# graehl/carmel

Hardware: AMD Instinct MI355X
Metric: arc-updates/sec (EM iterations/sec x derivation-lattice arcs swept per iteration) (higher is better)
Workload: dtype f64; 1 GPU; c4: synthetic 1000000-state / 9999990-arc WFST, 1000000 training pairs per GPU (random walks of 5-40 arcs), conditional normalisation, cached lattices; parallelism=corpus-sharded x1, none

## Files before the change

### carmel_amd/csrc/engine.cpp

```cpp
#include <hip/hip_runtime.h>
#include <chrono>
#include <cmath>
#include <cstdio>
#include <cstring>
#include <cstdlib>
#include <limits>
#include <string>
#include <thread>
#include <unordered_map>
#include <vector>
#include "engine.hpp"
#include "options.hpp"
#include "host/refhash.hpp"
#include "rng.hpp"
#include "unrolled_args.hpp"

int unrolled_try_build(carmel_hip_trainer* t, int host_threads, uint8_t* has_derivation, carmel_hip_lattice_stats* stats);
int gpu_build_lattices(carmel_hip_trainer* t, const BuildOptions& opt, uint8_t* has_derivation, carmel_hip_lattice_stats* stats,
                       bool& done);
int gpu_tables_for_host_layout(carmel_hip_trainer* t, const std::vector<uint32_t>& lane_arc, const std::vector<uint32_t>& wave_arc);
int carmel_hip_debug_lattice_fingerprint_impl(carmel_hip_trainer* t, uint64_t* out);
int build_run_tables(carmel_hip_trainer* t);
int exchange_weights_in(carmel_hip_trainer* t, ExchangePlan* xp, const TransArgs& T, bool need_x);
int exchange_counts_out(carmel_hip_trainer* t, ExchangePlan* xp, const TransArgs& T);
// ... 828 lines not shown
  T.b_src = t->t_b_src.p;
  T.t_pos = t->t_t_pos.p;
  T.t_src = t->t_t_src.p;
  T.a_off = t->t_a_off.p;
  T.tr_off = t->tr_off.p;
  T.tr_rel = t->tr_rel.p;
  T.tr_src = t->tr_src.p;
  T.br_off = t->br_off.p;
  T.br_rel = t->br_rel.p;
  T.br_src = t->br_src.p;
  T.use_runs = t->use_runs ? 1u : 0u;
  {
    const char* e = lib_opt("trans_scatter");
    T.scatter = e ? (uint32_t)atoi(e) : (t->use_runs ? 3u : 0u);
    if (t->lat.lane_fused) T.scatter &= ~2u;
  }
  T.x = t->t_x.p;
  T.xc = t->t_xc.p;
  T.logw = t->arc_logw.p;
  T.wcache = t->wcache.p;
  T.post = t->post.p;
  T.counts = t->counts_ptr();
  T.n_wcache = t->wcache.n;
  T.n_post = t->post.n;
  T.n_buckets = (uint32_t)t->t_buckets.n;
  T.n_tiles = t->t_tile_base.n ? (uint32_t)(t->t_tile_base.n - 1) : 0u;
  T.tile = t->lat.tile;
  T.bucket = t->lat.bucket;
  T.tile_first = T.tile_count = 0;
  T.bucket_first = 0;
  T.bucket_count = T.n_buckets;
  T.n_wtiles = 0;
  T.slack_bytes = (uint32_t)DEVBUF_SLACK;
}

__global__ __launch_bounds__(256) void lds_poison_kernel(unsigned* sink) {
  extern __shared__ unsigned lds_words[];
  const unsigned n = 160 * 1024 / 4 - 64;
  for (unsigned i = threadIdx.x; i < n; i += 256) lds_words[i] = 0xffffffffu;
  __syncthreads();
  if (lds_words[(threadIdx.x * 977u) % n] != 0xffffffffu) *sink = 1;
}
static int lds_poison(carmel_hip_trainer* t) {
  const int mode = lib_opt("poison") ? atoi(lib_opt("poison")) : 0;
  if (mode < 2) return CARMEL_HIP_OK;
  static bool attr = false;
  const int bytes = 160 * 1024 - 256;
  if (!attr) {
    HIPCHK(hipFuncSetAttribute((const void*)lds_poison_kernel, hipFuncAttributeMaxDynamicSharedMemorySize, bytes));
    attr = true;
  }
  hipLaunchKernelGGL(lds_poison_kernel, dim3(2048), dim3(256), bytes, t->stream, (unsigned*)t->maxchg.p);
  HIPCHK(hipGetLastError());
  HIPCHK(hipStreamSynchronize(t->stream));
  return CARMEL_HIP_OK;
}

int scalars_join(carmel_hip_trainer* t) {
  if (!t->scalars_pending) return CARMEL_HIP_OK;
  if (hipEventQuery(t->ev_join) != hipSuccess) HIPCHK(hipStreamWaitEvent(t->stream, t->ev_join, 0));
  t->scalars_pending = false;
  return CARMEL_HIP_OK;
}

__global__ void publish_kernel(const unsigned long long* src, unsigned long long* box, unsigned long long seq) {
  __hip_atomic_store(box, *src, __ATOMIC_RELAXED, __HIP_MEMORY_SCOPE_SYSTEM);
// ... 742 lines not shown
```

### carmel_amd/csrc/kernels.hip

```cpp
#include "kernels.hpp"
#include "sweep_math.hpp"
#include <algorithm>
#include <cstdio>
#include <cstdlib>

namespace carmel_hip {


__device__ __forceinline__ double lw_add(double a, double b) {
  if (a == NEG_INF) return b;
  if (b == NEG_INF) return a;
  double d = a - b;
  if (d > 36.0) return a;
  if (d < -36.0) return b;
  if (d < 0) return b + log1p(exp(d));
  return a + log1p(exp(-d));
}

__device__ __forceinline__ void atomic_add_f64(double* p, double v) {
  unsafeAtomicAdd(p, v);
}


#define LANE_W(r) (PRE ? wcache[(size_t)(((r).x >> LANE_POS_SHIFT) & LANE_POS_MAX) * 64] : logw[(r).y])
// ... 521 lines not shown
    f[s] = NEG_INF;
    bb[s] = NEG_INF;
  }
  f[st] = 0.0;
  for (uint32_t s = 0; s < ns; ++s) {
    for (uint32_t a = ooff[s]; a < ooff[s + 1]; ++a) {
      const uint2 r = oa[a];
      f[r.x] = lw_add(f[r.x], f[s] + A.logw[r.y]);
    }
  }
  const double prob = f[fin];
  A.pair_logprob[A.pair_id[d.pair_base]] = prob;
  const double lwt = A.pair_logw[d.pair_base];
  bb[fin] = 0.0;
  for (uint32_t s = ns; s-- > 0;) {
    for (uint32_t a = ioff[s]; a < ioff[s + 1]; ++a) {
      const uint2 r = ia[a];
      bb[r.x] = lw_add(bb[r.x], bb[s] + A.logw[r.y]);
    }
  }
  for (uint32_t s = 0; s < ns; ++s)
    for (uint32_t a = ooff[s]; a < ooff[s + 1]; ++a) {
      const uint2 r = oa[a];
      post[a] = (prob != NEG_INF) ? exp(A.logw[r.y] + f[s] + bb[r.x] + lwt - prob) : 0.0;
    }
}

#define SCALAR_BLOCKS 256
__global__ __launch_bounds__(256) void scalars_partial_kernel(const double* __restrict__ pair_logprob,
                                                              const double* __restrict__ pair_w, uint64_t n_pairs,
                                                              double* __restrict__ partial) {
  __shared__ double sh[3][4];
  double a = 0.0, b = 0.0, c = 0.0;
  for (uint64_t p = (uint64_t)blockIdx.x * 256 + threadIdx.x; p < n_pairs; p += (uint64_t)SCALAR_BLOCKS * 256) {
    const double w = pair_w[p];
    if (w < 0.0) continue;
    const double lp = pair_logprob[p];
    a += lp;
    b += lp * w;
    c += 1.0;
  }
  for (int o = 32; o > 0; o >>= 1) {
    a += __shfl_down(a, o, 64);
    b += __shfl_down(b, o, 64);
    c += __shfl_down(c, o, 64);
  }
  if ((threadIdx.x & 63) == 0) {
    sh[0][threadIdx.x >> 6] = a;
    sh[1][threadIdx.x >> 6] = b;
    sh[2][threadIdx.x >> 6] = c;
  }
  __syncthreads();
  if (threadIdx.x < 3) partial[blockIdx.x * 3 + threadIdx.x] = sh[threadIdx.x][0] + sh[threadIdx.x][1] + sh[threadIdx.x][2] + sh[threadIdx.x][3];
}
__global__ void scalars_final_kernel(const double* __restrict__ partial, double* __restrict__ scalars) {
  if (threadIdx.x < 3) {
    double v[4] = {0.0, 0.0, 0.0, 0.0};
    for (int k = 0; k < SCALAR_BLOCKS; k += 4)
      for (int j = 0; j < 4; ++j) v[j] += partial[(k + j) * 3 + threadIdx.x];
    scalars[threadIdx.x] = (v[0] + v[1]) + (v[2] + v[3]);
  } else if (threadIdx.x == 3)
    scalars[3] = 0.0;
}

#define COUNT_HOT 64
__global__ __launch_bounds__(256) void count_reduce_kernel(ReduceArgs R) {
  for (uint64_t a = (uint64_t)blockIdx.x * blockDim.x + threadIdx.x; a < R.n_arcs;
       a += (uint64_t)gridDim.x * blockDim.x) {
    const uint64_t j0 = R.arc_off[a], j1 = R.arc_off[a + 1];
    double c = 0.0;
    if (j1 - j0 <= COUNT_HOT)
      for (uint64_t j = j0; j < j1; ++j) c += R.post[R.slot_pos[j]];
    R.counts[a] = c;
// ... 330 lines not shown
                                     const double* arc_prior_w, const uint32_t* arc_chain, const uint64_t* chain_off,
                                     const uint64_t* chain_param, const uint32_t* param_group, uint64_t n_arcs) {
  for (uint64_t k = (uint64_t)blockIdx.x * blockDim.x + threadIdx.x; k < n_arcs; k += (uint64_t)gridDim.x * blockDim.x) {
    const double c = arc_counts[k] + (arc_prior_w ? arc_prior + arc_prior_w[k] : arc_prior);
    if (!(c > 0.0)) continue;
    const uint32_t ch = arc_chain[k];
    for (uint64_t j = chain_off[ch]; j < chain_off[ch + 1]; ++j) {
      const uint64_t p = chain_param[j];
      if (param_group[p] != 0u) atomic_add_f64(param_counts + p, c);
    }
  }
}

__global__ void add_f64_kernel(double* dst, const double* src, uint64_t n) {
  for (uint64_t k = (uint64_t)blockIdx.x * blockDim.x + threadIdx.x; k < n; k += (uint64_t)gridDim.x * blockDim.x) dst[k] += src[k];
}
__global__ void fill_f64_kernel(double* p, double v, uint64_t n) {
  for (uint64_t k = (uint64_t)blockIdx.x * blockDim.x + threadIdx.x; k < n; k += (uint64_t)gridDim.x * blockDim.x) p[k] = v;
}

#define TRANS_RUN_WORDS ((TRANS_TILE > TRANS_BUCKET ? TRANS_TILE : TRANS_BUCKET) / 32)
struct RunLds {
  uint32_t* r_src;
  uint32_t* mask;
  uint32_t* pref;
};
__device__ __forceinline__ RunLds run_lds(double* after_tile) {
  RunLds R;
  R.r_src = (uint32_t*)after_tile;
  R.mask = R.r_src + TRANS_RUN_CAP;
  R.pref = R.mask + TRANS_RUN_WORDS;
  return R;
}
__device__ __forceinline__ void run_stage(const RunLds& R, const uint16_t* __restrict__ rel, const uint32_t* __restrict__ src,
                                          uint32_t nr) {
  constexpr uint32_t WORDS = TRANS_RUN_WORDS, PER = WORDS / 64;
  for (uint32_t w = threadIdx.x; w < WORDS; w += 1024) R.mask[w] = 0u;
  __syncthreads();
  for (uint32_t r = threadIdx.x; r < nr; r += 1024) {
    const uint32_t first = rel[r];
    R.r_src[r] = src[r] - first;
    atomicOr(&R.mask[first >> 5], 1u << (first & 31u));
  }
  __syncthreads();
  if (threadIdx.x < 64) {
    uint32_t c[PER], tot = 0;
#pragma unroll
    for (uint32_t k = 0; k < PER; ++k) {
      c[k] = tot;
      tot += __popc(R.mask[threadIdx.x * PER + k]);
    }
    uint32_t inc = tot;
#pragma unroll
    for (int o = 1; o < 64; o <<= 1) {
      const uint32_t v = __shfl_up(inc, o, 64);
      if ((int)threadIdx.x >= o) inc += v;
    }
    const uint32_t before = inc - tot;
#pragma unroll
    for (uint32_t k = 0; k < PER; ++k) R.pref[threadIdx.x * PER + k] = before + c[k];
  }
  __syncthreads();
}
__device__ __forceinline__ uint32_t run_source(const RunLds& R, uint32_t i) {
  const uint32_t w = i >> 5;
  const uint32_t run = R.pref[w] + __popc(R.mask[w] & (0xffffffffu >> (31u - (i & 31u)))) - 1u;
  return R.r_src[run] + i;
}
template <bool SC, bool RL, int KB = TRANS_KB>
__global__ __launch_bounds__(1024) void trans_w_bucket_kernel(TransArgs T) {
  extern __shared__ __attribute__((aligned(16))) double lds[];
  const RunLds R = run_lds(lds + KB * 1024);
  uint32_t bloc = blockIdx.x;
  if (SC) {
    bloc = xcd_chunked(blockIdx.x, T.bucket_count);
    if (bloc >= T.bucket_count) return;
  }
  const uint32_t bucket = T.bucket_first + bloc;
  const TransBucket B = T.buckets[bucket];
  double w[KB];
#pragma unroll
  for (int k = 0; k < KB; ++k) {
    const uint32_t a = threadIdx.x + k * 1024;
    w[k] = a < B.n_arcs ? T.logw[B.arc_lo + a] : 0.0;
  }
  uint16_t ia[KB];
  uint32_t dst[KB];
#pragma unroll
  for (int k = 0; k < KB; ++k) {
    const uint32_t j = threadIdx.x + k * 1024;
    ia[k] = j < B.n_items ? T.b_arc[B.item_base + j] : (uint16_t)0;
    if (SC && !RL) dst[k] = j < B.n_items ? T.b_src[B.item_base + j] : 0u;
  }
#pragma unroll
  for (int k = 0; k < KB; ++k) lds[threadIdx.x + k * 1024] = w[k];
  if (SC && RL) {
    const uint32_t r0 = T.br_off[bucket];
    run_stage(R, T.br_rel + r0, T.br_src + r0, T.br_off[bucket + 1] - r0);
  } else
    __syncthreads();
#pragma unroll
  for (int k = 0; k < KB; ++k) {
    const uint32_t j = threadIdx.x + k * 1024;
    if (j < B.n_items) {
      if (SC)
        T.x[RL ? run_source(R, j) : dst[k]] = lds[ia[k]];
      else
        T.x[B.item_base + j] = lds[ia[k]];
    }
  }
}
#ifndef TRANS_TILE_WAVES
#define TRANS_TILE_WAVES 4
#endif
#ifndef TRANS_WB_WAVES
#define TRANS_WB_WAVES 4
#endif
template <bool RL, bool SQ>
__global__ __launch_bounds__(1024) __attribute__((amdgpu_waves_per_eu(TRANS_TILE_WAVES, TRANS_TILE_WAVES))) void trans_w_tile_kernel(TransArgs T) {
  extern __shared__ __attribute__((aligned(16))) double lds[];
  const RunLds R = run_lds(lds + TRANS_TILE);
  const uint32_t tloc = xcd_chunked(blockIdx.x, T.tile_count);
  if (tloc >= T.tile_count) return;
  const uint32_t tile = T.tile_first + tloc;
  const uint64_t p0 = (uint64_t)tile * T.tile;
  if (p0 >= T.n_wcache) return;
  const uint32_t np = (uint32_t)min((uint64_t)T.tile, T.n_wcache - p0);
#pragma unroll
  for (int k = 0; k < TRANS_KT; ++k) lds[threadIdx.x + k * 1024] = 0.0;
  if (RL && !SQ) {
    const uint32_t r0 = T.tr_off[tile];
    run_stage(R, T.tr_rel + r0, T.tr_src + r0, T.tr_off[tile + 1] - r0);
// ... 114 lines not shown
    if (threadIdx.x + k * NT < ni) lds[pos[k]] = v[k];
  __syncthreads();
#pragma unroll
  for (int k = 0; k < K; ++k) {
    const uint32_t q = threadIdx.x + k * NT;
    if (q < np) T.wcache[p0 + q] = lds[q];
  }
}
__global__ __launch_bounds__(TRANS_SMALL_THREADS) void trans_c_tile_small_kernel(TransArgs T) {
  __shared__ double lds[LANE_FUSED_TILE];
  constexpr int NT = TRANS_SMALL_THREADS, K = TRANS_SMALL_K;
  const uint32_t tile = T.tile_first + blockIdx.x;
  const uint64_t p0 = (uint64_t)tile * LANE_FUSED_TILE;
  const uint32_t np = p0 < T.n_post ? (uint32_t)min((uint64_t)LANE_FUSED_TILE, T.n_post - p0) : 0u;
  const uint64_t i0 = T.tile_base[tile];
  const uint32_t ni = (uint32_t)(T.tile_base[tile + 1] - i0);
  double v[K];
  uint16_t pos[K];
#pragma unroll
  for (int k = 0; k < K; ++k) {
    const uint32_t q = threadIdx.x + k * NT;
    v[k] = q < np ? T.post[p0 + q] : 0.0;
    pos[k] = q < ni ? T.t_pos[i0 + q] : (uint16_t)0;
  }
#pragma unroll
  for (int k = 0; k < K; ++k) lds[threadIdx.x + k * NT] = v[k];
  __syncthreads();
#pragma unroll
  for (int k = 0; k < K; ++k) {
    const uint32_t i = threadIdx.x + k * NT;
    if (i < ni) T.xc[i0 + i] = lds[pos[k]];
  }
}
template <bool RL, bool SQ, int KB = TRANS_KB>
__global__ __launch_bounds__(1024) void trans_c_bucket_kernel(TransArgs T) {
  extern __shared__ __attribute__((aligned(16))) double lds[];
  const RunLds R = run_lds(lds + KB * 1024);
  __shared__ double part[16];
  __shared__ uint32_t big[512];
  __shared__ uint32_t n_big;
  const uint32_t bloc = xcd_chunked(blockIdx.x, T.bucket_count);
  if (bloc >= T.bucket_count) return;
  const uint32_t bucket = T.bucket_first + bloc;
  const TransBucket B = T.buckets[bucket];
  uint16_t r0[KB], r1[KB];
  const bool single = (B.flags & TRANS_SINGLE) != 0;
#pragma unroll
  for (int k = 0; k < KB; ++k) {
    const uint32_t a = threadIdx.x + k * 1024;
    const bool ok = !single && a < B.n_arcs;
    r0[k] = ok ? T.a_off[B.arc_lo + a] : (uint16_t)0;
    r1[k] = (ok && a + 1 < B.n_arcs) ? T.a_off[B.arc_lo + a + 1] : (uint16_t)0;
  }
  {
    uint32_t src[KB];
    uint16_t rk[KB];
    double v[KB];
    if (RL && !SQ) {
      const uint32_t r0 = T.br_off[bucket];
      run_stage(R, T.br_rel + r0, T.br_src + r0, T.br_off[bucket + 1] - r0);
    }
#pragma unroll
    for (int k = 0; k < KB; ++k) {
      const uint32_t j = threadIdx.x + k * 1024;
      if (SQ)
        src[k] = 0u;
      else if (RL)
        src[k] = j < B.n_items ? run_source(R, j) : 0u;
      else
        src[k] = j < B.n_items ? T.b_src[B.item_base + j] : 0u;
      rk[k] = j < B.n_items ? T.b_rank[B.item_base + j] : (uint16_t)0;
    }
#pragma unroll
    for (int k = 0; k < KB; ++k) {
      if (SQ) {
        const uint32_t j = threadIdx.x + k * 1024;
        v[k] = j < B.n_items ? T.xc[B.item_base + j] : 0.0;
      } else
        v[k] = T.xc[src[k]];
    }
#pragma unroll
    for (int k = 0; k < KB; ++k)
      if (threadIdx.x + k * 1024 < B.n_items) lds[rk[k]] = v[k];
  }
  __syncthreads();
  if (single) {
    double v = 0.0;
    for (uint32_t j = threadIdx.x; j < B.n_items; j += 1024) v += lds[j];
    for (int o = 32; o > 0; o >>= 1) v += __shfl_down(v, o, 64);
    if ((threadIdx.x & 63) == 0) part[threadIdx.x >> 6] = v;
    __syncthreads();
    if (threadIdx.x == 0) {
      double tot = 0.0;
      for (int k = 0; k < 16; ++k) tot += part[k];
      if (B.flags & TRANS_SPLIT)
        atomic_add_f64(T.counts + B.arc_lo, tot);
      else
        T.counts[B.arc_lo] = tot;
    }
    return;
  }
  if (threadIdx.x == 0) n_big = 0;
  __syncthreads();
#pragma unroll
  for (int k = 0; k < KB; ++k) {
    const uint32_t a = threadIdx.x + k * 1024;
    if (a >= B.n_arcs) break;
    const uint32_t q0 = r0[k], q1 = a + 1 < B.n_arcs ? (uint32_t)r1[k] : B.n_items;
    if (q1 - q0 > 32) {
      const uint32_t q = atomicAdd(&n_big, 1u);
      if (q < 512) {
        big[q] = a;
        continue;
      }
    }
    double v = 0.0;
    for (uint32_t r = q0; r < q1; ++r) v += lds[r];
    T.counts[B.arc_lo + a] = v;
  }
  __syncthreads();
  const uint32_t nb = n_big < 512 ? n_big : 512;
  for (uint32_t q = threadIdx.x >> 6; q < nb; q += 16) {
    const uint32_t a = big[q];
    const uint32_t q0 = T.a_off[B.arc_lo + a], q1 = a + 1 < B.n_arcs ? (uint32_t)T.a_off[B.arc_lo + a + 1] : B.n_items;
    double v = 0.0;
    for (uint32_t r = q0 + (threadIdx.x & 63); r < q1; r += 64) v += lds[r];
    for (int o = 32; o > 0; o >>= 1) v += __shfl_down(v, o, 64);
    if ((threadIdx.x & 63) == 0) T.counts[B.arc_lo + a] = v;
  }
}
__global__ void zero_list_kernel(double* p, const uint32_t* idx, uint32_t n) {
  uint32_t k = blockIdx.x * blockDim.x + threadIdx.x;
  if (k < n) p[idx[k]] = 0.0;
}

static inline int grid_for(uint64_t n, int block) {
  uint64_t g = (n + block - 1) / block;
  if (g > 256ull * 16) g = 256ull * 16;
  if (g < 1) g = 1;
  return (int)g;
}

template <int R, int W, bool PRE, bool WIN = false, bool XC = false>
static hipError_t launch_lane_variant(const LaneArgs& A, unsigned grid, size_t lds, hipStream_t stream) {
  if (lds > 64 * 1024)
    (void)hipFuncSetAttribute((const void*)sweep_lane_kernel<R, W, PRE, Lse, WIN, XC>, hipFuncAttributeMaxDynamicSharedMemorySize, (int)lds);
  hipLaunchKernelGGL((sweep_lane_kernel<R, W, PRE, Lse, WIN, XC>), dim3(grid), dim3(64), lds, stream, A);
  return hipGetLastError();
}

hipError_t launch_lane_sweep(const LaneArgs& A0, const LatticeSet::LaneClass& lc, hipStream_t stream, bool fused) {
  LaneArgs A = A0;
  A.first_group = lc.first;
  A.lds_rows = lc.max_states;
  size_t lds = (size_t)lc.max_states * 64 * sizeof(double);
  if (fused) {
    if (!A.pre_weights || !A.xc || !A.xc_tile_base || !A.xc_t_pos) return hipErrorInvalidValue;
    lds += (size_t)LANE_FUSED_TILE * sizeof(double);
    if (lc.windowed) {
      if (!A.spill) return hipErrorInvalidValue;
      return launch_lane_variant<4, 2, true, true, true>(A, lc.count, lds, stream);
// ... 62 lines not shown
  } else if (lc.block == 64) {
    hipLaunchKernelGGL((sweep_bundle_kernel<64, true>), dim3(lc.count), dim3(64), lds, stream, A);
  } else if (lc.block == 256) {
    hipLaunchKernelGGL((sweep_bundle_kernel<256, true>), dim3(lc.count), dim3(256), lds, stream, A);
  } else {
    (void)hipFuncSetAttribute((const void*)sweep_bundle_kernel<1024, true>, hipFuncAttributeMaxDynamicSharedMemorySize,
                              (int)lds);
    hipLaunchKernelGGL((sweep_bundle_kernel<1024, true>), dim3(lc.count), dim3(1024), lds, stream, A);
  }
  return hipGetLastError();
}

#define TRANS_SET_LDS(K, BYTES) (void)hipFuncSetAttribute((const void*)K, hipFuncAttributeMaxDynamicSharedMemorySize, BYTES)
static void trans_lds_attr() {
  static unsigned char done_dev[64] = {0};
  int dev = 0;
  if (hipGetDevice(&dev) != hipSuccess || dev < 0 || dev >= 64) return;
  unsigned char& done = done_dev[dev];
  if (__atomic_load_n(&done, __ATOMIC_ACQUIRE)) return;
  const int lds = (int)(TRANS_TILE > TRANS_BUCKET ? TRANS_TILE : TRANS_BUCKET) * 8;
  const int lds_rl = lds + TRANS_RUN_LDS;
  TRANS_SET_LDS((trans_w_bucket_kernel<false, false>), lds);
  TRANS_SET_LDS((trans_w_bucket_kernel<true, false>), lds);
  TRANS_SET_LDS((trans_w_bucket_kernel<true, true>), lds_rl);
  TRANS_SET_LDS((trans_w_tile_kernel<false, false>), lds);
  TRANS_SET_LDS((trans_w_tile_kernel<true, false>), lds_rl);
  TRANS_SET_LDS((trans_w_tile_kernel<false, true>), lds);
  TRANS_SET_LDS((trans_c_tile_kernel<false, false>), lds);
  TRANS_SET_LDS((trans_c_tile_kernel<true, false>), lds);
  TRANS_SET_LDS((trans_c_tile_kernel<true, true>), lds_rl);
  TRANS_SET_LDS((trans_c_bucket_kernel<false, false>), lds);
  TRANS_SET_LDS((trans_c_bucket_kernel<true, false>), lds_rl);
  TRANS_SET_LDS((trans_c_bucket_kernel<false, true>), lds);
  {
    constexpr int KH = TRANS_KB / 2;
    TRANS_SET_LDS((trans_w_bucket_kernel<false, false, KH>), lds);
    TRANS_SET_LDS((trans_w_bucket_kernel<true, false, KH>), lds);
    TRANS_SET_LDS((trans_w_bucket_kernel<true, true, KH>), lds_rl);
    TRANS_SET_LDS((trans_c_bucket_kernel<false, false, KH>), lds);
    TRANS_SET_LDS((trans_c_bucket_kernel<true, false, KH>), lds_rl);
    TRANS_SET_LDS((trans_c_bucket_kernel<false, true, KH>), lds);
  }
  __atomic_store_n(&done, (unsigned char)1, __ATOMIC_RELEASE);
}
hipError_t launch_trans_w_bucket_range(const TransArgs& T0, uint32_t first, uint32_t count, hipStream_t stream) {
  trans_lds_attr();
  if (!T0.n_buckets || !count) return hipSuccess;
  TransArgs T = T0;
  T.bucket_first = first;
  T.bucket_count = count;
  const dim3 g8((count + 7) / 8 * 8);
  if (T.bucket == TRANS_BUCKET / 2) {
    constexpr int KH = TRANS_KB / 2;
    if (!(T.scatter & 1u))
      hipLaunchKernelGGL((trans_w_bucket_kernel<false, false, KH>), dim3(count), dim3(1024), KH * 1024 * 8, stream, T);
    else if (T.use_runs)
      hipLaunchKernelGGL((trans_w_bucket_kernel<true, true, KH>), g8, dim3(1024), KH * 1024 * 8 + TRANS_RUN_LDS, stream, T);
    else
      hipLaunchKernelGGL((trans_w_bucket_kernel<true, false, KH>), g8, dim3(1024), KH * 1024 * 8, stream, T);
    return hipGetLastError();
  }
  if (T.bucket != TRANS_BUCKET) return hipErrorInvalidValue;
  if (!(T.scatter & 1u))
    hipLaunchKernelGGL((trans_w_bucket_kernel<false, false>), dim3(count), dim3(1024), TRANS_BUCKET * 8, stream, T);
  else if (T.use_runs)
    hipLaunchKernelGGL((trans_w_bucket_kernel<true, true>), g8, dim3(1024), TRANS_BUCKET * 8 + TRANS_RUN_LDS, stream, T);
  else
    hipLaunchKernelGGL((trans_w_bucket_kernel<true, false>), g8, dim3(1024), TRANS_BUCKET * 8, stream, T);
  return hipGetLastError();
}
hipError_t launch_trans_w_bucket(const TransArgs& T, hipStream_t stream) { return launch_trans_w_bucket_range(T, 0, T.n_buckets, stream); }
hipError_t launch_trans_w_tiles(const TransArgs& T0, uint32_t tile_first, uint32_t tile_count, hipStream_t stream) {
  trans_lds_attr();
  if (!T0.n_buckets || !tile_count) return hipSuccess;
  TransArgs T = T0;
  T.tile_first = tile_first;
// ... 28 lines not shown
    return hipGetLastError();
  }
  if (T.tile != TRANS_TILE && T.tile != TILE_SWEEP_TILE) return hipErrorInvalidValue;
  if (!(T.scatter & 2u))
    hipLaunchKernelGGL((trans_c_tile_kernel<false, false>), dim3(tile_count), dim3(1024), TRANS_TILE * 8, stream, T);
  else if (T.use_runs)
    hipLaunchKernelGGL((trans_c_tile_kernel<true, true>), g8, dim3(1024), TRANS_TILE * 8 + TRANS_RUN_LDS, stream, T);
  else
    hipLaunchKernelGGL((trans_c_tile_kernel<true, false>), g8, dim3(1024), TRANS_TILE * 8, stream, T);
  return hipGetLastError();
}
hipError_t launch_zero_list(double* p, const uint32_t* idx, uint32_t n, hipStream_t stream) {
  if (n) hipLaunchKernelGGL(zero_list_kernel, dim3((n + 255) / 256), dim3(256), 0, stream, p, idx, n);
  return hipGetLastError();
}
hipError_t launch_trans_c_bucket_range(const TransArgs& T0, uint32_t first, uint32_t count, hipStream_t stream) {
  trans_lds_attr();
  if (!T0.n_buckets || !count) return hipSuccess;
  TransArgs T = T0;
  T.bucket_first = first;
  T.bucket_count = count;
  const dim3 g8((count + 7) / 8 * 8);
  if (T.bucket == TRANS_BUCKET / 2) {
    constexpr int KH = TRANS_KB / 2;
    if (T.scatter & 2u)
      hipLaunchKernelGGL((trans_c_bucket_kernel<false, true, KH>), g8, dim3(1024), KH * 1024 * 8, stream, T);
    else if (T.use_runs)
      hipLaunchKernelGGL((trans_c_bucket_kernel<true, false, KH>), g8, dim3(1024), KH * 1024 * 8 + TRANS_RUN_LDS, stream, T);
    else
      hipLaunchKernelGGL((trans_c_bucket_kernel<false, false, KH>), g8, dim3(1024), KH * 1024 * 8, stream, T);
    return hipGetLastError();
  }
  if (T.bucket != TRANS_BUCKET) return hipErrorInvalidValue;
  if (T.scatter & 2u)
    hipLaunchKernelGGL((trans_c_bucket_kernel<false, true>), g8, dim3(1024), TRANS_BUCKET * 8, stream, T);
  else if (T.use_runs)
    hipLaunchKernelGGL((trans_c_bucket_kernel<true, false>), g8, dim3(1024), TRANS_BUCKET * 8 + TRANS_RUN_LDS, stream, T);
  else
    hipLaunchKernelGGL((trans_c_bucket_kernel<false, false>), g8, dim3(1024), TRANS_BUCKET * 8, stream, T);
  return hipGetLastError();
}
hipError_t launch_trans_c_bucket(const TransArgs& T, const uint32_t* split_arcs, uint32_t n_split, hipStream_t stream) {
  if (!T.n_buckets) return hipSuccess;
  hipError_t e = launch_zero_list(T.counts, split_arcs, n_split, stream);
  if (e != hipSuccess) return e;
  return launch_trans_c_bucket_range(T, 0, T.n_buckets, stream);
}
__global__ void gather_idx_kernel(double* small, const double* src, const uint32_t* idx, uint32_t n) {
  const uint32_t k = blockIdx.x * blockDim.x + threadIdx.x;
  if (k < n) small[k] = src[idx[k]];
}
__global__ void scatter_idx_kernel(double* dst, const double* small, const uint32_t* idx, uint32_t n) {
  const uint32_t k = blockIdx.x * blockDim.x + threadIdx.x;
  if (k < n) dst[idx[k]] = small[k];
}
hipError_t launch_gather_idx(double* small, const double* src, const uint32_t* idx, uint32_t n, hipStream_t stream) {
  if (n) hipLaunchKernelGGL(gather_idx_kernel, dim3((n + 255) / 256), dim3(256), 0, stream, small, src, idx, n);
  return hipGetLastError();
}
hipError_t launch_scatter_idx(double* dst, const double* small, const uint32_t* idx, uint32_t n, hipStream_t stream) {
  if (n) hipLaunchKernelGGL(scatter_idx_kernel, dim3((n + 255) / 256), dim3(256), 0, stream, dst, small, idx, n);
  return hipGetLastError();
}

hipError_t launch_count_reduce(const ReduceArgs& R, hipStream_t stream) {
  if (!R.n_arcs) return hipSuccess;
// ... 103 lines not shown
```

### carmel_amd/csrc/kernels.hpp

```cpp
#pragma once
#include <hip/hip_runtime.h>
#include <stdint.h>
#include "lattice.hpp"

namespace carmel_hip {

struct LaneArgs {
  const LaneGroup* groups;
  const uint2* fwd;
  const uint32_t* fwdx;
  const uint32_t* bwd;
  const uint32_t* rec2;
  const uint32_t* chain;
  const uint32_t* tile_chain;
  const uint32_t* lane_pair;
  const uint32_t* lane_nstates;
  const double* lane_logw;
  const double* logw;
  double* post;
  double* wcache;
  double* scalars;
  double* pair_logprob;
  double* spill;
  uint32_t first_group;
// ... 57 lines not shown
struct TransArgs {
  const TransBucket* buckets;
  const uint64_t* tile_base;
  const uint16_t* b_arc;
  const uint16_t* b_rank;
  const uint32_t* b_src;
  const uint16_t* t_pos;
  const uint32_t* t_src;
  const uint16_t* a_off;
  double* x;
  double* xc;
  const double* logw;
  double* wcache;
  const double* post;
  double* counts;
  uint64_t n_wcache, n_post;
  uint32_t n_buckets, n_tiles;
  uint32_t n_wtiles;
  const uint32_t* tr_off;
  const uint16_t* tr_rel;
  const uint32_t* tr_src;
  const uint32_t* br_off;
  const uint16_t* br_rel;
  const uint32_t* br_src;
  uint32_t use_runs;
  uint32_t scatter;
  uint32_t tile;
  uint32_t bucket;
  uint32_t tile_first, tile_count;
  uint32_t bucket_first, bucket_count;
  uint32_t slack_bytes;
  const uint32_t* zero_list = nullptr;
  uint32_t n_zero = 0;
};

#define TRANS_RUN_CAP 4096
#define TRANS_RUN_LDS (TRANS_RUN_CAP * 4 + 4096)
#define MSTEP_BIG_GROUP 48
#define MSTEP_PARTIALS 2048
#define MSTEP_MAX_RANGES 17
#define MSTEP_WIDE_SLOTS 512
#define MSTEP_WIDE_SHARDS 32
#define MSTEP_WIDE_TICKETS (16 * (MSTEP_WIDE_SHARDS + 1))
struct MstepArgs {
  double* logw;
  const double* lw_src;
  double* old_logw;
  const double* counts;
  const double* prior;
  const uint32_t* group;
  const uint32_t* norm_of;
  const double* add_count;
  const uint64_t* group_off;
  const uint64_t* norm_perm;
  const uint64_t* big_groups;
  uint64_t n_groups, n_big;
  double* gscale;
  unsigned long long* max_partial;
  unsigned long long* max_change_bits;
  int all_grouped;
  uint32_t window_span;
  double* glocked;
  const uint32_t* tie_of;
  double* tie_tab;
  uint64_t n_ties;
  uint64_t n;
  uint32_t block_first;
// ... 57 lines not shown
```

### carmel_amd/csrc/options.cpp

```cpp
#include "options.hpp"
#include <cstdlib>
#include <cstring>
#include <mutex>
#include <string>
#include "../../include/carmel_hip.h"

namespace carmel_hip {
namespace {
const char* const kKeys[] = {
    "timing",
    "lane_states", "tile_sweep", "lane_fused", "transpose", "lane_chunks", "lane_window", "lane_window_min", "wave_ring", "wave_min_width",
    "gpu_build", "wave_gather", "wave_xc", "tile_gather", "device_tables", "trans_scatter", "trans_runs", "lane_fused_kernel",
    "tile_sweep_kernel", "mailbox", "poison", "lane_trace", "exchange_sparse", "mstep_wide",
    "dense", "unrolled", "unrolled_ragged",
    "gibbs_chains", "gibbs_own_cap", "gibbs_workgroup", "gibbs_clk", "gibbs_reg", "gibbs_lane", "forest_sweep", "forest_ldswalk", "forest_multi",
    "forest_nohash", "forest_trace", "forest_exact_host", "forest_exact_clk", "forest_logdomain", "forest_gcol", "forest_gather",
    "decode_lds", "decode_chunk_bytes"};
constexpr int kN = (int)(sizeof kKeys / sizeof kKeys[0]);
const char* volatile g_val[kN];
std::mutex g_mu;
int find(const char* key) {
  for (int i = 0; i < kN; ++i)
    if (!std::strcmp(kKeys[i], key)) return i;
  return -1;
}
}
const char* lib_opt(const char* key) {
  const int i = find(key);
  return i < 0 ? nullptr : g_val[i];
}
bool lib_opt_off(const char* key) {
  const char* v = lib_opt(key);
  return v && std::atoi(v) == 0;
}
}

extern "C" {
int carmel_hip_set_option(const char* key, const char* value) {
  using namespace carmel_hip;
  if (!key) return CARMEL_HIP_ERR_ARG;
  const int i = find(key);
  if (i < 0) return CARMEL_HIP_ERR_ARG;
  std::lock_guard<std::mutex> lk(g_mu);
  if (!value)
    g_val[i] = nullptr;
  else {
// ... 12 lines not shown
```

Baseline: 51.67 billion arc-updates/s.

## Make count-transpose bucket kernel persistent with next-bucket prefetch

Turns the trans_c_bucket kernel into a persistent grid-stride walk over buckets, sized by default to the CU count, and prefetches the next bucket's descriptor and run offsets while the current one is processed. Run-table loads are issued into registers before LDS staging, a_off pairs are read as one 32-bit load, and the scalar reduction kernel unrolls 16 loads per thread. The aim is to hide descriptor and global load latency and cut block launch overhead. The cost is fewer resident blocks and extra barriers per bucket, and load balance may suffer when buckets vary in size.

After: 53.02 billion arc-updates/s (median of 6 runs). +2.6%, better.

```diff
diff --git a/carmel_amd/csrc/engine.cpp b/carmel_amd/csrc/engine.cpp
--- a/carmel_amd/csrc/engine.cpp
+++ b/carmel_amd/csrc/engine.cpp
@@ -884,6 +884,8 @@
   T.bucket_count = T.n_buckets;
   T.n_wtiles = 0;
   T.slack_bytes = (uint32_t)DEVBUF_SLACK;
+  T.bucket_walk = TRANS_WALK_AUTO;
+  if (const char* e = lib_opt("trans_bucket_walk")) T.bucket_walk = (uint32_t)std::max(0, atoi(e));
 }
 
 __global__ __launch_bounds__(256) void lds_poison_kernel(unsigned* sink) {
diff --git a/carmel_amd/csrc/kernels.hip b/carmel_amd/csrc/kernels.hip
--- a/carmel_amd/csrc/kernels.hip
+++ b/carmel_amd/csrc/kernels.hip
@@ -577,13 +577,23 @@
                                                               double* __restrict__ partial) {
   __shared__ double sh[3][4];
   double a = 0.0, b = 0.0, c = 0.0;
-  for (uint64_t p = (uint64_t)blockIdx.x * 256 + threadIdx.x; p < n_pairs; p += (uint64_t)SCALAR_BLOCKS * 256) {
-    const double w = pair_w[p];
-    if (w < 0.0) continue;
-    const double lp = pair_logprob[p];
-    a += lp;
-    b += lp * w;
-    c += 1.0;
+  constexpr int SCALAR_ROUNDS = 16;
+  constexpr uint64_t STRIDE = (uint64_t)SCALAR_BLOCKS * 256;
+  for (uint64_t p0 = (uint64_t)blockIdx.x * 256 + threadIdx.x; p0 < n_pairs; p0 += STRIDE * SCALAR_ROUNDS) {
+    double w[SCALAR_ROUNDS], lp[SCALAR_ROUNDS];
+#pragma unroll
+    for (int k = 0; k < SCALAR_ROUNDS; ++k) {
+      const uint64_t p = p0 + k * STRIDE;
+      w[k] = p < n_pairs ? pair_w[p] : -1.0;
+      lp[k] = p < n_pairs ? pair_logprob[p] : 0.0;
+    }
+#pragma unroll
+    for (int k = 0; k < SCALAR_ROUNDS; ++k) {
+      if (w[k] < 0.0) continue;
+      a += lp[k];
+      b += lp[k] * w[k];
+      c += 1.0;
+    }
   }
   for (int o = 32; o > 0; o >>= 1) {
     a += __shfl_down(a, o, 64);
@@ -980,10 +990,29 @@
   R.pref = R.mask + TRANS_RUN_WORDS;
   return R;
 }
+__device__ __forceinline__ void run_prefix(const RunLds& R) {
+  constexpr uint32_t WORDS = TRANS_RUN_WORDS, PER = WORDS / 64;
+  if (threadIdx.x < 64) {
+    uint32_t c[PER], tot = 0;
+#pragma unroll
+    for (uint32_t k = 0; k < PER; ++k) {
+      c[k] = tot;
+      tot += __popc(R.mask[threadIdx.x * PER + k]);
+    }
+    uint32_t inc = tot;
+#pragma unroll
+    for (int o = 1; o < 64; o <<= 1) {
+      const uint32_t v = __shfl_up(inc, o, 64);
+      if ((int)threadIdx.x >= o) inc += v;
+    }
+    const uint32_t before = inc - tot;
+#pragma unroll
+    for (uint32_t k = 0; k < PER; ++k) R.pref[threadIdx.x * PER + k] = before + c[k];
+  }
+}
 __device__ __forceinline__ void run_stage(const RunLds& R, const uint16_t* __restrict__ rel, const uint32_t* __restrict__ src,
                                           uint32_t nr) {
-  constexpr uint32_t WORDS = TRANS_RUN_WORDS, PER = WORDS / 64;
-  for (uint32_t w = threadIdx.x; w < WORDS; w += 1024) R.mask[w] = 0u;
+  for (uint32_t w = threadIdx.x; w < TRANS_RUN_WORDS; w += 1024) R.mask[w] = 0u;
   __syncthreads();
   for (uint32_t r = threadIdx.x; r < nr; r += 1024) {
     const uint32_t first = rel[r];
@@ -991,29 +1020,86 @@
     atomicOr(&R.mask[first >> 5], 1u << (first & 31u));
   }
   __syncthreads();
-  if (threadIdx.x < 64) {
-    uint32_t c[PER], tot = 0;
-#pragma unroll
-    for (uint32_t k = 0; k < PER; ++k) {
-      c[k] = tot;
-      tot += __popc(R.mask[threadIdx.x * PER + k]);
-    }
-    uint32_t inc = tot;
-#pragma unroll
-    for (int o = 1; o < 64; o <<= 1) {
-      const uint32_t v = __shfl_up(inc, o, 64);
-      if ((int)threadIdx.x >= o) inc += v;
-    }
-    const uint32_t before = inc - tot;
-#pragma unroll
-    for (uint32_t k = 0; k < PER; ++k) R.pref[threadIdx.x * PER + k] = before + c[k];
-  }
+  run_prefix(R);
+  __syncthreads();
+}
+#define RUN_K (TRANS_RUN_CAP / 1024)
+struct RunRegs {
+  uint32_t first[RUN_K], src[RUN_K];
+};
+__device__ __forceinline__ RunRegs run_request(const uint16_t* __restrict__ rel, const uint32_t* __restrict__ src, uint32_t nr) {
+  RunRegs q;
+#pragma unroll
+  for (int k = 0; k < RUN_K; ++k) {
+    const uint32_t r = threadIdx.x + k * 1024;
+    q.first[k] = r < nr ? (uint32_t)rel[r] : 0u;
+    q.src[k] = r < nr ? src[r] : 0u;
+  }
+  return q;
+}
+__device__ __forceinline__ void run_stage(const RunLds& R, const RunRegs& q, uint32_t nr) {
+  for (uint32_t w = threadIdx.x; w < TRANS_RUN_WORDS; w += 1024) R.mask[w] = 0u;
+  __syncthreads();
+#pragma unroll
+  for (int k = 0; k < RUN_K; ++k) {
+    const uint32_t r = threadIdx.x + k * 1024;
+    if (r < nr) {
+      R.r_src[r] = q.src[k] - q.first[k];
+      atomicOr(&R.mask[q.first[k] >> 5], 1u << (q.first[k] & 31u));
+    }
+  }
+  __syncthreads();
+  run_prefix(R);
   __syncthreads();
 }
 __device__ __forceinline__ uint32_t run_source(const RunLds& R, uint32_t i) {
   const uint32_t w = i >> 5;
   const uint32_t run = R.pref[w] + __popc(R.mask[w] & (0xffffffffu >> (31u - (i & 31u)))) - 1u;
   return R.r_src[run] + i;
+}
+__device__ __forceinline__ uint32_t bw_zero() {
+  uint32_t z = 0;
+  asm volatile("" : "+v"(z));
+  return z;
+}
+__device__ __forceinline__ uint32_t bw_opaque(uint32_t v) {
+  asm volatile("" : "+v"(v));
+  return v;
+}
+__device__ __forceinline__ uint32_t bw_sc(uint32_t v) { return __builtin_amdgcn_readfirstlane(v); }
+struct BucketWalk {
+  uint32_t bucket;
+  bool ok;
+};
+__device__ __forceinline__ BucketWalk bucket_walk_at(const TransArgs& T, uint32_t vidx) {
+  BucketWalk w;
+  const uint32_t bloc = xcd_chunked(vidx, T.bucket_count);
+  w.ok = bloc < T.bucket_count && (vidx >> 3) < (T.bucket_count + 7) / 8;
+  w.bucket = T.bucket_first + (w.ok ? bloc : 0u);
+  return w;
+}
+struct BucketAhead {
+  TransBucket B;
+  uint32_t r0, r1;
+};
+template <bool RUNS>
+__device__ __forceinline__ BucketAhead bucket_request(const TransArgs& T, uint32_t bucket, uint32_t z) {
+  BucketAhead a;
+  a.B = T.buckets[bucket + z];
+  a.r0 = RUNS ? T.br_off[bucket + z] : 0u;
+  a.r1 = RUNS ? T.br_off[bucket + 1 + z] : 0u;
+  return a;
+}
+__device__ __forceinline__ BucketAhead bw_uniform(const BucketAhead& v) {
+  BucketAhead a;
+  a.B.item_base = ((uint64_t)bw_sc((uint32_t)(v.B.item_base >> 32)) << 32) | bw_sc((uint32_t)v.B.item_base);
+  a.B.n_items = bw_sc(v.B.n_items);
+  a.B.arc_lo = bw_sc(v.B.arc_lo);
+  a.B.n_arcs = bw_sc(v.B.n_arcs);
+  a.B.flags = bw_sc(v.B.flags);
+  a.r0 = bw_sc(v.r0);
+  a.r1 = bw_sc(v.r1);
+  return a;
 }
 template <bool SC, bool RL, int KB = TRANS_KB>
 __global__ __launch_bounds__(1024) void trans_w_bucket_kernel(TransArgs T) {
@@ -1026,6 +1112,11 @@
   }
   const uint32_t bucket = T.bucket_first + bloc;
   const TransBucket B = T.buckets[bucket];
+  uint32_t run0 = 0, nr = 0;
+  if (SC && RL) {
+    run0 = T.br_off[bucket];
+    nr = T.br_off[bucket + 1] - run0;
+  }
   double w[KB];
 #pragma unroll
   for (int k = 0; k < KB; ++k) {
@@ -1040,12 +1131,13 @@
     ia[k] = j < B.n_items ? T.b_arc[B.item_base + j] : (uint16_t)0;
     if (SC && !RL) dst[k] = j < B.n_items ? T.b_src[B.item_base + j] : 0u;
   }
+  RunRegs runs;
+  if (SC && RL) runs = run_request(T.br_rel + run0, T.br_src + run0, nr);
 #pragma unroll
   for (int k = 0; k < KB; ++k) lds[threadIdx.x + k * 1024] = w[k];
-  if (SC && RL) {
-    const uint32_t r0 = T.br_off[bucket];
-    run_stage(R, T.br_rel + r0, T.br_src + r0, T.br_off[bucket + 1] - r0);
-  } else
+  if (SC && RL)
+    run_stage(R, runs, nr);
+  else
     __syncthreads();
 #pragma unroll
   for (int k = 0; k < KB; ++k) {
@@ -1226,101 +1318,122 @@
     if (i < ni) T.xc[i0 + i] = lds[pos[k]];
   }
 }
-template <bool RL, bool SQ, int KB = TRANS_KB>
+template <bool RL, bool SQ, int KB = TRANS_KB, bool WALK = false>
 __global__ __launch_bounds__(1024) void trans_c_bucket_kernel(TransArgs T) {
   extern __shared__ __attribute__((aligned(16))) double lds[];
   const RunLds R = run_lds(lds + KB * 1024);
   __shared__ double part[16];
   __shared__ uint32_t big[512];
   __shared__ uint32_t n_big;
-  const uint32_t bloc = xcd_chunked(blockIdx.x, T.bucket_count);
-  if (bloc >= T.bucket_count) return;
-  const uint32_t bucket = T.bucket_first + bloc;
-  const TransBucket B = T.buckets[bucket];
-  uint16_t r0[KB], r1[KB];
-  const bool single = (B.flags & TRANS_SINGLE) != 0;
-#pragma unroll
-  for (int k = 0; k < KB; ++k) {
-    const uint32_t a = threadIdx.x + k * 1024;
-    const bool ok = !single && a < B.n_arcs;
-    r0[k] = ok ? T.a_off[B.arc_lo + a] : (uint16_t)0;
-    r1[k] = (ok && a + 1 < B.n_arcs) ? T.a_off[B.arc_lo + a + 1] : (uint16_t)0;
-  }
-  {
-    uint32_t src[KB];
-    uint16_t rk[KB];
-    double v[KB];
-    if (RL && !SQ) {
-      const uint32_t r0 = T.br_off[bucket];
-      run_stage(R, T.br_rel + r0, T.br_src + r0, T.br_off[bucket + 1] - r0);
-    }
+  const uint32_t z = WALK ? bw_zero() : 0u;
+  uint32_t vidx = blockIdx.x;
+  BucketWalk cur = bucket_walk_at(T, vidx);
+  if (!cur.ok) return;
+  BucketAhead A = bw_uniform(bucket_request<RL && !SQ>(T, cur.bucket, z));
+  for (;;) {
+    const TransBucket B = A.B;
+    const uint32_t tx = WALK ? bw_opaque(threadIdx.x) : threadIdx.x;
+    BucketWalk nxt = cur;
+    nxt.ok = false;
+    BucketAhead raw;
+    if (WALK) {
+      nxt = bucket_walk_at(T, vidx + gridDim.x);
+      raw = bucket_request<RL && !SQ>(T, nxt.bucket, z);
+    }
+    uint32_t r01[KB];
+    const bool single = (B.flags & TRANS_SINGLE) != 0;
 #pragma unroll
     for (int k = 0; k < KB; ++k) {
-      const uint32_t j = threadIdx.x + k * 1024;
-      if (SQ)
-        src[k] = 0u;
-      else if (RL)
-        src[k] = j < B.n_items ? run_source(R, j) : 0u;
-      else
-        src[k] = j < B.n_items ? T.b_src[B.item_base + j] : 0u;
-      rk[k] = j < B.n_items ? T.b_rank[B.item_base + j] : (uint16_t)0;
-    }
-#pragma unroll
-    for (int k = 0; k < KB; ++k) {
-      if (SQ) {
-        const uint32_t j = threadIdx.x + k * 1024;
-        v[k] = j < B.n_items ? T.xc[B.item_base + j] : 0.0;
-      } else
-        v[k] = T.xc[src[k]];
-    }
-#pragma unroll
-    for (int k = 0; k < KB; ++k)
-      if (threadIdx.x + k * 1024 < B.n_items) lds[rk[k]] = v[k];
-  }
-  __syncthreads();
-  if (single) {
-    double v = 0.0;
-    for (uint32_t j = threadIdx.x; j < B.n_items; j += 1024) v += lds[j];
-    for (int o = 32; o > 0; o >>= 1) v += __shfl_down(v, o, 64);
-    if ((threadIdx.x & 63) == 0) part[threadIdx.x >> 6] = v;
+      const uint32_t a = tx + k * 1024;
+      r01[k] = 0u;
+      if (!single && a < B.n_arcs) __builtin_memcpy(&r01[k], T.a_off + B.arc_lo + a, 4);
+    }
+    {
+      uint32_t src[KB];
+      uint16_t rk[KB];
+      double v[KB];
+#pragma unroll
+      for (int k = 0; k < KB; ++k) {
+        const uint32_t j = tx + k * 1024;
+        rk[k] = j < B.n_items ? T.b_rank[B.item_base + j] : (uint16_t)0;
+      }
+      if (RL && !SQ) {
+        const RunRegs runs = run_request(T.br_rel + A.r0, T.br_src + A.r0, A.r1 - A.r0);
+        run_stage(R, runs, A.r1 - A.r0);
+      }
+#pragma unroll
+      for (int k = 0; k < KB; ++k) {
+        const uint32_t j = tx + k * 1024;
+        if (SQ)
+          src[k] = 0u;
+        else if (RL)
+          src[k] = j < B.n_items ? run_source(R, j) : 0u;
+        else
+          src[k] = j < B.n_items ? T.b_src[B.item_base + j] : 0u;
+      }
+#pragma unroll
+      for (int k = 0; k < KB; ++k) {
+        if (SQ) {
+          const uint32_t j = tx + k * 1024;
+          v[k] = j < B.n_items ? T.xc[B.item_base + j] : 0.0;
+        } else
+          v[k] = T.xc[src[k]];
+      }
+#pragma unroll
+      for (int k = 0; k < KB; ++k)
+        if (tx + k * 1024 < B.n_items) lds[rk[k]] = v[k];
+    }
+    if (threadIdx.x == 0) n_big = 0;
     __syncthreads();
-    if (threadIdx.x == 0) {
-      double tot = 0.0;
-      for (int k = 0; k < 16; ++k) tot += part[k];
-      if (B.flags & TRANS_SPLIT)
-        atomic_add_f64(T.counts + B.arc_lo, tot);
-      else
-        T.counts[B.arc_lo] = tot;
-    }
-    return;
-  }
-  if (threadIdx.x == 0) n_big = 0;
-  __syncthreads();
-#pragma unroll
-  for (int k = 0; k < KB; ++k) {
-    const uint32_t a = threadIdx.x + k * 1024;
-    if (a >= B.n_arcs) break;
-    const uint32_t q0 = r0[k], q1 = a + 1 < B.n_arcs ? (uint32_t)r1[k] : B.n_items;
-    if (q1 - q0 > 32) {
-      const uint32_t q = atomicAdd(&n_big, 1u);
-      if (q < 512) {
-        big[q] = a;
-        continue;
+    BucketAhead An = A;
+    if (WALK) An = bw_uniform(raw);
+    if (single) {
+      double v = 0.0;
+      for (uint32_t j = threadIdx.x; j < B.n_items; j += 1024) v += lds[j];
+      for (int o = 32; o > 0; o >>= 1) v += __shfl_down(v, o, 64);
+      if ((threadIdx.x & 63) == 0) part[threadIdx.x >> 6] = v;
+      __syncthreads();
+      if (threadIdx.x == 0) {
+        double tot = 0.0;
+        for (int k = 0; k < 16; ++k) tot += part[k];
+        if (B.flags & TRANS_SPLIT)
+          atomic_add_f64(T.counts + B.arc_lo, tot);
+        else
+          T.counts[B.arc_lo] = tot;
       }
-    }
-    double v = 0.0;
-    for (uint32_t r = q0; r < q1; ++r) v += lds[r];
-    T.counts[B.arc_lo + a] = v;
-  }
-  __syncthreads();
-  const uint32_t nb = n_big < 512 ? n_big : 512;
-  for (uint32_t q = threadIdx.x >> 6; q < nb; q += 16) {
-    const uint32_t a = big[q];
-    const uint32_t q0 = T.a_off[B.arc_lo + a], q1 = a + 1 < B.n_arcs ? (uint32_t)T.a_off[B.arc_lo + a + 1] : B.n_items;
-    double v = 0.0;
-    for (uint32_t r = q0 + (threadIdx.x & 63); r < q1; r += 64) v += lds[r];
-    for (int o = 32; o > 0; o >>= 1) v += __shfl_down(v, o, 64);
-    if ((threadIdx.x & 63) == 0) T.counts[B.arc_lo + a] = v;
+    } else {
+#pragma unroll
+      for (int k = 0; k < KB; ++k) {
+        const uint32_t a = tx + k * 1024;
+        if (a < B.n_arcs) {
+          const uint32_t q0 = r01[k] & 0xffffu, q1 = a + 1 < B.n_arcs ? r01[k] >> 16 : B.n_items;
+          uint32_t q = 512u;
+          if (q1 - q0 > 32) q = atomicAdd(&n_big, 1u);
+          if (q < 512u)
+            big[q] = a;
+          else {
+            double v = 0.0;
+            for (uint32_t r = q0; r < q1; ++r) v += lds[r];
+            T.counts[B.arc_lo + a] = v;
+          }
+        }
+      }
+      __syncthreads();
+      const uint32_t nb = n_big < 512 ? n_big : 512;
+      for (uint32_t q = threadIdx.x >> 6; q < nb; q += 16) {
+        const uint32_t a = big[q];
+        const uint32_t q0 = T.a_off[B.arc_lo + a], q1 = a + 1 < B.n_arcs ? (uint32_t)T.a_off[B.arc_lo + a + 1] : B.n_items;
+        double v = 0.0;
+        for (uint32_t r = q0 + (threadIdx.x & 63); r < q1; r += 64) v += lds[r];
+        for (int o = 32; o > 0; o >>= 1) v += __shfl_down(v, o, 64);
+        if ((threadIdx.x & 63) == 0) T.counts[B.arc_lo + a] = v;
+      }
+    }
+    if (!WALK || !nxt.ok) break;
+    __syncthreads();
+    A = An;
+    cur = nxt;
+    vidx += gridDim.x;
   }
 }
 __global__ void zero_list_kernel(double* p, const uint32_t* idx, uint32_t n) {
@@ -1449,6 +1562,9 @@
   TRANS_SET_LDS((trans_c_bucket_kernel<false, false>), lds);
   TRANS_SET_LDS((trans_c_bucket_kernel<true, false>), lds_rl);
   TRANS_SET_LDS((trans_c_bucket_kernel<false, true>), lds);
+  TRANS_SET_LDS((trans_c_bucket_kernel<false, false, TRANS_KB, true>), lds);
+  TRANS_SET_LDS((trans_c_bucket_kernel<true, false, TRANS_KB, true>), lds_rl);
+  TRANS_SET_LDS((trans_c_bucket_kernel<false, true, TRANS_KB, true>), lds);
   {
     constexpr int KH = TRANS_KB / 2;
     TRANS_SET_LDS((trans_w_bucket_kernel<false, false, KH>), lds);
@@ -1459,6 +1575,24 @@
     TRANS_SET_LDS((trans_c_bucket_kernel<false, true, KH>), lds);
   }
   __atomic_store_n(&done, (unsigned char)1, __ATOMIC_RELEASE);
+}
+static uint32_t trans_walk_grid(const TransArgs& T, uint32_t count) {
+  if (!T.bucket_walk || T.bucket != TRANS_BUCKET) return 0;
+  uint32_t cap = T.bucket_walk;
+  if (cap == TRANS_WALK_AUTO) {
+    static int dev_cus[64] = {0};
+    int dev = 0;
+    if (hipGetDevice(&dev) != hipSuccess || dev < 0 || dev >= 64) return 0;
+    if (!__atomic_load_n(&dev_cus[dev], __ATOMIC_ACQUIRE)) {
+      hipDeviceProp_t prop;
+      if (hipGetDeviceProperties(&prop, dev) != hipSuccess) return 0;
+      __atomic_store_n(&dev_cus[dev], prop.multiProcessorCount > 8 ? prop.multiProcessorCount / 8 * 8 : 8, __ATOMIC_RELEASE);
+    }
+    cap = (uint32_t)__atomic_load_n(&dev_cus[dev], __ATOMIC_ACQUIRE);
+    if (cap >= (count + 7) / 8 * 8) return 0;
+  } else
+    cap = cap > (1u << 20) ? (1u << 20) : (cap + 7) / 8 * 8;
+  return std::min(cap, (count + 7) / 8 * 8);
 }
 hipError_t launch_trans_w_bucket_range(const TransArgs& T0, uint32_t first, uint32_t count, hipStream_t stream) {
   trans_lds_attr();
@@ -1553,6 +1687,15 @@
     return hipGetLastError();
   }
   if (T.bucket != TRANS_BUCKET) return hipErrorInvalidValue;
+  if (const uint32_t gw = trans_walk_grid(T, count)) {
+    if (T.scatter & 2u)
+      hipLaunchKernelGGL((trans_c_bucket_kernel<false, true, TRANS_KB, true>), dim3(gw), dim3(1024), TRANS_BUCKET * 8, stream, T);
+    else if (T.use_runs)
+      hipLaunchKernelGGL((trans_c_bucket_kernel<true, false, TRANS_KB, true>), dim3(gw), dim3(1024), TRANS_BUCKET * 8 + TRANS_RUN_LDS, stream, T);
+    else
+      hipLaunchKernelGGL((trans_c_bucket_kernel<false, false, TRANS_KB, true>), dim3(gw), dim3(1024), TRANS_BUCKET * 8, stream, T);
+    return hipGetLastError();
+  }
   if (T.scatter & 2u)
     hipLaunchKernelGGL((trans_c_bucket_kernel<false, true>), g8, dim3(1024), TRANS_BUCKET * 8, stream, T);
   else if (T.use_runs)
diff --git a/carmel_amd/csrc/kernels.hpp b/carmel_amd/csrc/kernels.hpp
--- a/carmel_amd/csrc/kernels.hpp
+++ b/carmel_amd/csrc/kernels.hpp
@@ -113,7 +113,9 @@
   uint32_t slack_bytes;
   const uint32_t* zero_list = nullptr;
   uint32_t n_zero = 0;
-};
+  uint32_t bucket_walk = 0xffffffffu;
+};
+#define TRANS_WALK_AUTO 0xffffffffu
 
 #define TRANS_RUN_CAP 4096
 #define TRANS_RUN_LDS (TRANS_RUN_CAP * 4 + 4096)
diff --git a/carmel_amd/csrc/options.cpp b/carmel_amd/csrc/options.cpp
--- a/carmel_amd/csrc/options.cpp
+++ b/carmel_amd/csrc/options.cpp
@@ -11,7 +11,7 @@
     "timing",
     "lane_states", "tile_sweep", "lane_fused", "transpose", "lane_chunks", "lane_window", "lane_window_min", "wave_ring", "wave_min_width",
     "gpu_build", "wave_gather", "wave_xc", "tile_gather", "device_tables", "trans_scatter", "trans_runs", "lane_fused_kernel",
-    "tile_sweep_kernel", "mailbox", "poison", "lane_trace", "exchange_sparse", "mstep_wide",
+    "tile_sweep_kernel", "mailbox", "poison", "lane_trace", "exchange_sparse", "mstep_wide", "trans_bucket_walk",
     "dense", "unrolled", "unrolled_ragged",
     "gibbs_chains", "gibbs_own_cap", "gibbs_workgroup", "gibbs_clk", "gibbs_reg", "gibbs_lane", "forest_sweep", "forest_ldswalk", "forest_multi",
     "forest_nohash", "forest_trace", "forest_exact_host", "forest_exact_clk", "forest_logdomain", "forest_gcol", "forest_gather",
```
